# CentaureaHO/CTC-VR

Hardware: AMD Instinct MI355X
Metric: audio-frames/sec, streaming RNN-T greedy decode (higher is better)
Workload: dtype bf16x3; 1 GPU; configs[1]: batch=64/GPU synthetic 10 s 80-dim fbank, streaming chunk=16 (online_rnnt_decode.py semantics), greedy decode, whole-utterance call (tokens identical to the per-chunk API); streams_per_gpu=64, chunk_frames=16, chunks=62, weights=seeded synthetic (seed 0, blank_bias 12.0), parallelism=streams sharded x1, no data-path collective

## Files before the change

ctc-vr_amd/csrc/api_lifecycle.hip.inc:

```

int rnnt_abi_version(void) { return 3; }

const char* rnnt_last_error(const rnnt_ctx* ctx) { return ctx ? ctx->err.c_str() : "null context"; }

int rnnt_create(const rnnt_config* cfg, rnnt_ctx** out) {
    if (!cfg || !out) return RNNT_ERR_ARG;
    *out = nullptr;
    rnnt_ctx* ctx = new rnnt_ctx();
    ctx->cfg = *cfg;
    *out = ctx;
    if (cfg->max_streams < 1 || cfg->max_chunk_frames < 7 || cfg->max_cache_frames < 1 || cfg->max_cache_frames > RNNT_PE_LEN ||
        cfg->max_enc_frames < 1 || cfg->max_tokens < 1 || cfg->vocab_size < 2 || cfg->blank_id < 0 || cfg->blank_id >= cfg->vocab_size ||
        cfg->n_steps < 1 || cfg->max_beam < 0 || cfg->max_beam > 64)
        return fail(ctx, RNNT_ERR_ARG, "rnnt_create: bad config");
    HIPCHK(hipSetDevice(cfg->device));
    if (const char* ng = getenv("RNNT_NO_GRAPH")) ctx->use_graphs = (ng[0] == '1') ? 0 : 1;
    if (const char* pe = getenv("RNNT_PERSISTENT")) ctx->use_persistent = (pe[0] == '0') ? 0 : 1;
    if (const char* me = getenv("RNNT_DEC_MULTI")) ctx->use_multi = (me[0] == '0') ? 0 : 1;
    HIPCHK(hipDeviceGetAttribute(&ctx->n_cus, hipDeviceAttributeMultiprocessorCount, cfg->device));
    if (const char* ae = getenv("RNNT_ATTN_STREAM")) ctx->attn_stream = (ae[0] == '0') ? 0 : 1;
    if (const char* be = getenv("RNNT_BEAM_CHAIN")) ctx->use_beam_chain = (be[0] == '0') ? 0 : 1;
    if (const char* pg = getenv("RNNT_PREFIX_GROUP")) ctx->prefix_group = pg[0] == '1' ? 1 : (pg[0] == '4' ? 4 : 0);
    if (const char* fu = getenv("RNNT_FUSED")) ctx->use_fused = atoi(fu);
    if (const char* fe = getenv("RNNT_FUSE_AFTER_NORM")) ctx->fuse_after_norm = (fe[0] == '0') ? 0 : 1;
    if (const char* me = getenv("RNNT_WF_MERGE")) { const int m = atoi(me); ctx->wf_merge = m < 1 ? 1 : (m > WF_MERGE_MAX ? WF_MERGE_MAX : m); }
    if (const char* le = getenv("RNNT_LM")) ctx->use_lm = (le[0] == '0') ? 0 : 1;
    if (const char* ae2 = getenv("RNNT_AS")) ctx->use_as = (ae2[0] == '0') ? 0 : 1;
    if (const char* e_ = getenv("RNNT_LM_PW2_HEAD")) ctx->lm_pw2_head = atoi(e_);
    if (const char* e_ = getenv("RNNT_LM_FFN_MERGE")) ctx->lm_ffn_merge = atoi(e_);
    if (const char* e_ = getenv("RNNT_LM_SIDE")) ctx->lm_side = atoi(e_);
    if (const char* e_ = getenv("RNNT_LM_QKV_TAIL")) ctx->lm_qkv_tail = atoi(e_);
    if (const char* e_ = getenv("RNNT_LM_OUT_CHAIN")) ctx->lm_out_chain = atoi(e_);
    if (const char* e_ = getenv("RNNT_ATTN_BF")) ctx->attn_bf = atoi(e_);
    if (const char* e_ = getenv("RNNT_ATTN_RESIDENT")) ctx->attn_resident = atoi(e_);
    if (const char* e_ = getenv("RNNT_CONV1_FUSE")) ctx->conv1_fuse = atoi(e_);
    if (const char* se = getenv("RNNT_WF_SUB_ASYNC")) ctx->wf_sub_async = (se[0] == '0') ? 0 : 1;
    const int B = cfg->max_streams;
    ctx->slot = std::vector<PoolSlot>((size_t)B);
    ctx->hs_buf = std::vector<DevBuf<float>>((size_t)B);
    ctx->tmax = sub_len(cfg->max_chunk_frames);
    ctx->t1max = sub1_len(cfg->max_chunk_frames);
    ctx->cap = RNNT_LORDER + WF_MERGE_MAX * ctx->tmax;
    ctx->tcap = cfg->max_cache_frames;
    ctx->fcap = cfg->max_enc_frames;
    ctx->fstride = ctx->fcap + 1;
    ctx->vpad = (cfg->vocab_size + 31) / 32 * 32;
    const size_t M = (size_t)B * ctx->tmax;
    int rc;
#define ALLOC(p, n) if ((rc = reserve(ctx, ctx->p, (size_t)(n)))) return rc
    ALLOC(y1, (size_t)B * ctx->t1max * RNNT_F1 * D);
    ALLOC(y2, M * RNNT_FSUB * D);
    ALLOC(x, M * D);
    ALLOC(hbuf, M * FF);
    ALLOC(qbuf, M * D);
    ALLOC(abuf, M * D);
    ALLOC(dbuf, M * D);
    ALLOC(kcache, (size_t)L * B * ctx->tcap * D);
    ALLOC(vcache, (size_t)L * B * ctx->tcap * D);
    ALLOC(gring, (size_t)L * B * ctx->cap * D);
    ALLOC(xring, (size_t)L * B * ctx->cap * D);
    ALLOC(encbuf, (size_t)B * ctx->fstride * D);
    ALLOC(encp, (size_t)B * ctx->fstride * D);
    ALLOC(h, (size_t)2 * B * D); ALLOC(c, (size_t)2 * B * D); ALLOC(sel, B); ALLOC(key, B);
    ALLOC(pred, (size_t)B * D); ALLOC(z, (size_t)B * D); ALLOC(logits, (size_t)B * ctx->vpad);
    ALLOC(tok, B); ALLOC(fidx, B); ALLOC(nsym, B); ALLOC(count, B); ALLOC(tokens, (size_t)B * cfg->max_tokens);
    ALLOC(n_active, 4); ALLOC(klen, B); ALLOC(dec_ctrl, 32);
    ALLOC(gm_dbg, 16);
    ALLOC(gm_x1, (size_t)2 * B * GM_PARTS * GM_X1);
    ALLOC(gm_xa, (size_t)2 * B * GM_PARTS * 2 * GREEDY_KF);
    if (cfg->max_beam > 0) {
        ctx->max_rows = B * cfg->max_beam;
        const size_t R = ctx->max_rows, NS = cfg->n_steps, KB = cfg->max_beam;
        ALLOC(pool[0], R * (NS + 1) * 512); ALLOC(pool[1], R * (NS + 1) * 512);
        ALLOC(bpred, R * D); ALLOC(bz, R * D); ALLOC(blogits, R * ctx->vpad);
        ALLOC(b_blank, R * NS); ALLOC(b_toplp, R * NS * KB); ALLOC(b_toptok, R * NS * KB);
        ALLOC(b_tok, R); ALLOC(b_frame, R); ALLOC(b_active, R); ALLOC(b_steps, R); ALLOC(b_srcrow, R); ALLOC(b_srcstep, R);
    }
    ALLOC(scratch, std::max((size_t)L * RNNT_H * ctx->tcap * 128, (size_t)B * ctx->fstride * D));
    ALLOC(pinned, 16);
#undef ALLOC
    HIPCHK(hipMemset(ctx->encbuf, 0, (size_t)B * ctx->fstride * D * sizeof(float)));
    HIPCHK(hipMemset(ctx->encp, 0, (size_t)B * ctx->fstride * D * sizeof(float)));
    return RNNT_OK;
}

void rnnt_destroy(rnnt_ctx* ctx) {
    if (ctx) delete ctx;
}

int64_t rnnt_live_device_bytes(void) { return live_device_bytes.load(); }

int rnnt_load_tensor(rnnt_ctx* ctx, const char* name, const float* host_data, int32_t ndim, const int64_t* dims) {
    if (!ctx || !name || ndim < 0 || ndim > 8) return fail(ctx, RNNT_ERR_ARG, "rnnt_load_tensor: bad argument");
    std::string n(name);
    if (n.find("num_batches_tracked") != std::string::npos) return RNNT_OK;
    if (!host_data) return fail(ctx, RNNT_ERR_ARG, "rnnt_load_tensor(%s): null data", name);
    HostTensor t;
    size_t cnt = 1;
    for (int i = 0; i < ndim; ++i) {
        if (dims[i] < 0) return fail(ctx, RNNT_ERR_SHAPE, "rnnt_load_tensor(%s): negative dim", name);
        t.dims.push_back(dims[i]);
        cnt *= (size_t)dims[i];
    }
    t.data.assign(host_data, host_data + cnt);
    ctx->host[n] = std::move(t);
    ctx->finalized = false;
    return RNNT_OK;
}

int rnnt_load_packed(rnnt_ctx* ctx, const float* blob, int64_t n_floats, int32_t on_device, int32_t n_tensors, const char* const* names,
                     const int32_t* ndims, const int64_t* dims_flat) {
    if (!ctx || !blob || !names || !ndims || !dims_flat || n_floats < 0 || n_tensors < 1) return fail(ctx, RNNT_ERR_ARG, "rnnt_load_packed: bad argument");
    std::vector<float> host;
    const float* src = blob;
    if (on_device) {
        HIPCHK(hipSetDevice(ctx->cfg.device));
        host.resize((size_t)n_floats);
        HIPCHK(hipMemcpy(host.data(), blob, (size_t)n_floats * sizeof(float), hipMemcpyDeviceToHost));
        src = host.data();
    }
// ... 365 lines not shown
```

ctc-vr_amd/csrc/host_decode.hip.inc:

```

namespace {

GreedyState greedy_state(rnnt_ctx* ctx) {
    return GreedyState{ctx->tok, ctx->fidx, ctx->nsym, ctx->count, ctx->tokens, ctx->sel, ctx->key, ctx->n_active, ctx->pinned + 8};
}

int greedy_steps_raw(rnnt_ctx* ctx, hipStream_t s, int n) {
    const int B = ctx->n_streams, V = ctx->cfg.vocab_size;
    const long long bs = (long long)ctx->cfg.max_streams * D;
    GreedyState st = greedy_state(ctx);
    int rc;
    for (int it = 0; it < n; ++it) {
        hipLaunchKernelGGL(greedy_decide, dim3(1), dim3(64), 0, s, B, ctx->cfg.blank_id, ctx->cfg.n_steps, ctx->cfg.max_tokens, 0, st);
        LAUNCHCHK("greedy_decide");
        GemmP g1 = plain_gemm(ctx->h, D, ctx->whh_il, D, nullptr, ctx->h, D, B, 4 * D, D, EPI_LSTM);
        g1.X = ctx->egate; g1.I = ctx->tok; g1.X2 = ctx->c; g1.Y2 = ctx->c;
        g1.Asel = ctx->sel; g1.asel_stride = bs; g1.asel_invert = 0;
        g1.act_idx = ctx->fidx; g1.act_lim = ctx->n_active + 2;
        if ((rc = launch_gemm(ctx, s, &g1, 1, TAG_LSTM))) return rc;
        GemmP g3 = plain_gemm(ctx->h, D, ctx->wjc, D, ctx->bjc, ctx->z, D, B, D, D, EPI_TANH_ADD);
        g3.Asel = ctx->sel; g3.asel_stride = bs; g3.asel_invert = 1;
        g3.X = ctx->encp; g3.I = ctx->fidx; g3.x_n = 1; g3.x_s0 = (long long)ctx->fstride * D; g3.x_s1 = D;
        g3.act_idx = ctx->fidx; g3.act_lim = ctx->n_active + 2;
        if ((rc = launch_gemm(ctx, s, &g3, 1, TAG_JOINT_TANH))) return rc;
// ... 32 lines not shown
    e = hipGraphInstantiate(&exec, graph, nullptr, nullptr, 0);
    (void)hipGraphDestroy(graph);
    if (e != hipSuccess) return fail(ctx, RNNT_ERR_HIP, "hipGraphInstantiate failed: %s", hipGetErrorString(e));
    ctx->dec_graphs.push_back({ctx->n_streams, n, exec});
    HIPCHK(hipGraphLaunch(exec, s));
    ctx->launches += 4 * n;
    return RNNT_OK;
}

int greedy_drain(rnnt_ctx* ctx, hipStream_t s, int n_frames, int done_steps) {
    hipLaunchKernelGGL(fill_i32, dim3(1), dim3(64), 0, s, ctx->n_active + 2, n_frames, 1LL);
    LAUNCHCHK("fill_i32");
    const int max_steps = (n_frames - ctx->frames_decoded) * (ctx->cfg.n_steps + 1) + 8;
    int rc;
    while (true) {
        hipLaunchKernelGGL(greedy_decide, dim3(1), dim3(64), 0, s, ctx->n_streams, ctx->cfg.blank_id, ctx->cfg.n_steps, ctx->cfg.max_tokens, 1,
                           greedy_state(ctx));
        LAUNCHCHK("greedy_decide");
        HIPCHK(hipMemcpyAsync(ctx->pinned, ctx->n_active, sizeof(int), hipMemcpyDeviceToHost, s));
        HIPCHK(hipStreamSynchronize(s));
        if (ctx->pinned[0] <= 0) break;
        if (done_steps > max_steps) return fail(ctx, RNNT_ERR_STATE, "greedy decode did not terminate");
        static const int dstep = getenv("RNNT_DRAIN_STEPS") ? atoi(getenv("RNNT_DRAIN_STEPS")) : 4;
        if ((rc = greedy_steps(ctx, s, dstep, n_frames))) return rc;
        done_steps += dstep;
    }
    return RNNT_OK;
}


DecP dec_params(const rnnt_ctx* ctx, int n_total, int n_steps_override, const int* nlim, const int* slots, int n_rows) {
    DecP d{};
    d.whh = ctx->whh_il; d.egate = ctx->egate; d.wjc = ctx->wjc; d.bjc = ctx->bjc; d.wout = ctx->wout; d.bout = ctx->bout;
    d.encp = ctx->encp; d.h = ctx->h; d.c = ctx->c; d.sel = ctx->sel; d.tok = ctx->tok; d.fidx = ctx->fidx; d.nsym = ctx->nsym;
    d.count = ctx->count; d.tokens = ctx->tokens; d.ctrl = ctx->dec_ctrl;
    d.fstride_f = (long long)ctx->fstride * D; d.bstride = (long long)ctx->cfg.max_streams * D;
    d.B = slots ? n_rows : ctx->n_streams; d.vocab = ctx->cfg.vocab_size; d.blank = ctx->cfg.blank_id;
    d.n_steps = n_steps_override > 0 ? n_steps_override : ctx->cfg.n_steps;
    d.max_tokens = ctx->cfg.max_tokens; d.n_total = n_total; d.nlim = nlim; d.slots = slots;
    d.timeout_ticks = 500000000ll;
    return d;
}

bool multi_decoder_ok(const rnnt_ctx* ctx, int rows) {
    return ctx->use_multi && GM_PARTS * rows <= ctx->n_cus && (ctx->cfg.vocab_size + GM_PARTS - 1) / GM_PARTS <= 128;
}

int launch_multi_decoder(rnnt_ctx* ctx, hipStream_t s, const DecP& common) {
    static const bool gdbg = getenv("RNNT_GM_DBG") != nullptr;
    const int B = common.B, rows_per = (common.vocab + GM_PARTS - 1) / GM_PARTS;
    const DecMP d{common, ctx->gm_x1, ctx->gm_xa, rows_per, gdbg ? ctx->gm_dbg : nullptr};
    HIPCHK(hipMemsetAsync(ctx->gm_x1, 0, (size_t)2 * B * GM_PARTS * GM_X1 * sizeof(unsigned long long), s));
    HIPCHK(hipMemsetAsync(ctx->gm_xa, 0, (size_t)2 * B * GM_PARTS * 2 * GREEDY_KF * sizeof(unsigned long long), s));
    const size_t lds = ((size_t)rows_per * GM_WLD + 4 * D + GREEDY_KF * D + 16 * GREEDY_KF + GM_PARTS * 2 * GREEDY_KF + 8 + GREEDY_KF * 4 * 128) * sizeof(float);
    { const int rc_attr = ensure_dyn_lds(ctx, reinterpret_cast<const void*>(&greedy_multi<GREEDY_KF>), 160 * 1024); if (rc_attr) return rc_attr; }
    hipLaunchKernelGGL(greedy_multi<GREEDY_KF>, dim3((unsigned)((B + 7) / 8 * 8 * GM_PARTS)), dim3(512), lds, s, d);
    LAUNCHCHK("greedy_multi");
    return RNNT_OK;
}

int launch_persistent_decoder(rnnt_ctx* ctx, hipStream_t s, int n_total, int n_steps_override = 0, const int* nlim = nullptr,
                              const int* slots = nullptr, int n_rows = 0) {
    const DecP d = dec_params(ctx, n_total, n_steps_override, nlim, slots, n_rows);
    if (multi_decoder_ok(ctx, d.B)) return launch_multi_decoder(ctx, s, d);
    hipLaunchKernelGGL(greedy_stream<GREEDY_KF>, dim3(d.B), dim3(512), 0, s, d);
    LAUNCHCHK("greedy_stream");
    return RNNT_OK;
}

int init_decoder_ctrl(rnnt_ctx* ctx, hipStream_t s, int frames_ready) {
    hipLaunchKernelGGL(fill_i32, dim3(1), dim3(64), 0, s, ctx->dec_ctrl, 0, 32LL);
    LAUNCHCHK("fill_i32");
    hipLaunchKernelGGL(publish_frames, dim3(1), dim3(1), 0, s, ctx->dec_ctrl, frames_ready);
    LAUNCHCHK("publish_frames");
    return RNNT_OK;
}

int probe_overlap(rnnt_ctx* ctx, hipStream_t s, hipStream_t s2) {
    hipLaunchKernelGGL(fill_i32, dim3(1), dim3(64), 0, s, ctx->dec_ctrl, 0, 32LL);
    LAUNCHCHK("fill_i32");
    HIPCHK(hipStreamSynchronize(s));
    hipLaunchKernelGGL(probe_overlap_wait, dim3(1), dim3(1), 0, s2, ctx->dec_ctrl, 2000000LL);
    LAUNCHCHK("probe_overlap_wait");
    hipLaunchKernelGGL(publish_frames, dim3(1), dim3(1), 0, s, ctx->dec_ctrl, 1);
    LAUNCHCHK("publish_frames");
    HIPCHK(hipStreamSynchronize(s2));
    HIPCHK(hipStreamSynchronize(s));
    int r[2] = {0, 0};
    HIPCHK(hipMemcpy(r, ctx->dec_ctrl, sizeof(r), hipMemcpyDeviceToHost));
    ctx->overlap_ok = r[1] ? 1 : 0;
    if (!ctx->overlap_ok)
        fprintf(stderr, "[rnnt] kernels of two HIP streams do not overlap here (serialising profiler or shared hardware queue): "
                        "the resident decoder is replaced by launched evaluation batches\n");
    return RNNT_OK;
}

int finish_persistent_decoder(rnnt_ctx* ctx, hipStream_t s) {
    HIPCHK(hipMemcpyAsync(ctx->pinned + 12, ctx->dec_ctrl, 4 * sizeof(int), hipMemcpyDeviceToHost, s));
    HIPCHK(hipStreamSynchronize(s));
    ctx->greedy_steps += ctx->pinned[14];
    if (getenv("RNNT_GM_DBG") && multi_decoder_ok(ctx, ctx->n_streams)) {
        long long t[16];
        (void)hipMemcpy(t, ctx->gm_dbg, sizeof(t), hipMemcpyDeviceToHost);
        const double ev = t[8] > 0 ? (double)t[8] : 1.0, sy = t[9] > 0 ? (double)t[9] : 1.0;
        fprintf(stderr, "[greedy_multi] stream 0: %lld passes, %lld symbols; us per pass: frames %.2f, decide-tail %.2f, z+logits %.2f, wait XA %.2f; "
                        "us per symbol: W_hh %.2f, cell+W_c %.2f, wait X1 %.2f\n",
                t[8], t[9], t[0] / ev / 100.0, t[6] / ev / 100.0, t[4] / ev / 100.0, t[5] / ev / 100.0, t[1] / sy / 100.0, t[2] / sy / 100.0, t[3] / sy / 100.0);
    }
    if (ctx->pinned[13] != 0) return fail(ctx, RNNT_ERR_STATE, "persistent decoder gave up (code %d: 1 = frame wait, 2 = greedy_multi exchange wait)", ctx->pinned[13]);
    return RNNT_OK;
}

int decode_resident(rnnt_ctx* ctx, hipStream_t s, int n_total, const int* nlim = nullptr, const int* slots = nullptr, int n_rows = 0, int n_steps = 0) {
    int rc;
    if ((rc = init_decoder_ctrl(ctx, s, n_total))) return rc;
    if ((rc = launch_persistent_decoder(ctx, s, n_total, n_steps, nlim, slots, n_rows))) return rc;
    return finish_persistent_decoder(ctx, s);
}

}
```

ctc-vr_amd/csrc/rnnt_api.hip:

```cpp
#include "rnnt_kernels.hip.h"
#include "../../include/rnnt_hip.h"

#include <climits>
#include <cmath>
#include <cstdarg>
#include <cstdio>
#include <chrono>
#include <cstdlib>
#include <cstring>
#include <functional>
#include <map>
#include <string>
#include <unordered_map>
#include <algorithm>
#include <array>
#include <atomic>
#include <vector>

namespace {

constexpr int D = RNNT_D, FF = RNNT_FF, L = RNNT_L, DK = RNNT_DK;
constexpr int BIG = INT_MAX;

struct LayerW {
// ... 94 lines not shown
    PinnedBuf<int> host;
    hipEvent_t ev = nullptr;
    ~CallTab() { if (ev) (void)hipEventDestroy(ev); }
    operator int*() const { return dev.p; }
};

enum WfType { WF_FFN1M, WF_FFN2M, WF_QKV, WF_OUT, WF_PW1, WF_PW2, WF_FFN1, WF_FFN2, WF_ATTN, WF_DW, WF_LN, WF_BLOCK_FRONT, WF_BLOCK_BACK };

}

struct rnnt_ctx {
    rnnt_config cfg;
    std::string err;
    std::map<std::string, HostTensor> host;
    bool finalized = false;
    int numerics = 0;

    DevBuf<float> blob;
    DevBuf<unsigned short> blob_hi, blob_lo;
    DevBuf<uint4> fuse_w;
    DevBuf<LayerDev> layers_dev;
    const uint4* conv2_wp = nullptr;
    DevBuf<unsigned char> joint_wfrag;
    DevBuf<int> joint_counter;
    std::map<const void*, int> dyn_lds;
    std::vector<LayerDev> layers_host;
    int use_as = 1;
    int use_fused = 1;
    DevBuf<FuseItem> wf_ftab;
    int wf_fused_plan = 0;
    LayerW lw[L];
    DevBuf<float> ptab[L];
    const float *conv1_wt, *conv1_b, *conv2_w, *conv2_b, *emb_w, *emb_b, *pe, *after_g, *after_b;
    const float *ln_conv_g_all, *ln_conv_b_all, *glu0;
    const float *whh_il, *wih_il, *b_lstm_il, *pred_embed, *wpr, *bpr, *wenc, *benc, *wpf, *bpf, *wout, *bout;
    DevBuf<float> egate;

    int tmax = 0, t1max = 0, cap = 0, tcap = 0, fcap = 0, fstride = 0, vpad = 0;
    DevBuf<float> y1, y2, x, hbuf, qbuf, abuf, dbuf;
    DevBuf<float> kcache, vcache, gring, xring;
    DevBuf<float> encbuf, encp;
    DevBuf<float> h, c, pred, z, logits;
    DevBuf<int> tok, fidx, nsym, count, tokens, n_active, klen, sel;
    DevBuf<unsigned long long> key;
    DevBuf<int> dec_ctrl;
    int use_persistent = 1;
    int attn_stream = 1;
    int fuse_after_norm = 1;
    int overlap_ok = -1;
    int use_multi = 1;
    int n_cus = 0;
    DevBuf<unsigned long long> gm_x1, gm_xa;
    DevBuf<long long> gm_dbg;
    const float *wjc = nullptr, *bjc = nullptr;
    const float *wctc = nullptr, *bctc = nullptr;
    int max_rows = 0;
    DevBuf<float> pool[2], bpred, bz, blogits, b_blank, b_toplp;
    DevBuf<int> b_tok, b_frame, b_active, b_steps, b_toptok, b_srcrow, b_srcstep;
    int pool_cur = 0;
    PinnedBuf<int> pinned;
    DevBuf<float> scratch;

    int n_streams = 0;
    SlotPos pos{0, 0, 0};
    int frames_buffered = 0, frames_decoded = 0;
    int64_t launches = 0, greedy_steps = 0;
    std::vector<PoolSlot> slot;
    bool pool_mode = false;
    CallTab pool_tab;
    int gemm_m_cap = 0;
    DevBuf<float> wf_x, wf_h, wf_q, wf_a, wf_d, wf_y1, wf_y2;
    int wf_slab = 0;
    DevBuf<int> wf_starts;
    DevBuf<GemmP> wf_gtab; DevBuf<AttnP> wf_atab; DevBuf<DwP> wf_dtab; DevBuf<LnP> wf_ltab;
    hipStream_t dec_stream = nullptr;
    hipStream_t sub_stream = nullptr;
    int wf_sub_async = 1;
    int wf_merge = 2;
    struct WfLaunch { WfType type; int off, n, maxM, maxT2; };
    std::vector<WfLaunch> wf_seq;
    std::vector<std::array<int, 13>> wf_lstart;
    std::vector<int> wf_sc_first, wf_key;
    std::vector<hipEvent_t> ev_pool;
    int use_lm = 1;
    int lm_pw2_head = 2;
    int lm_ffn_merge = 0;
    int lm_qkv_tail = 1, lm_out_chain = 1;
    int lm_side = 1;
    int attn_bf = 1;
    int attn_resident = 1;
    int conv1_fuse = 1;
    DevBuf<float> lm_x, lm_h, lm_q, lm_a, lm_d, lm_g, lm_y1, lm_y2;
    DevBuf<float> lm_y1b, lm_y2b;
    hipEvent_t sub_ev[2] = {nullptr, nullptr};
    DevBuf<float> rg_fb, rg_xt;
    DevBuf<int2> rg_ent;
    DevBuf<LmBlock> lm_blocks;
    std::vector<LmBlock> lm_blocks_host;
    std::vector<int> lm_key;
    DevBuf<LmResHdr> lm_rhdr;
    DevBuf<LmRow> lm_rrows;
    std::vector<LmResHdr> lm_rhdr_host;
    std::vector<LmRow> lm_rrows_host;
    int lm_res_ok = 0, lm_res_stride = 0;
    struct Hyp { std::vector<int> tokens; double log_prob; };
    std::vector<std::vector<Hyp>> beams;
// ... 93 lines not shown
```

ctc-vr_amd/csrc/rnnt_decode.hip.h:

```cpp
#pragma once

struct GreedyState {
    int* tok;
    int* fidx;
    int* nsym;
    int* count;
    int* tokens;
    int* sel;
    unsigned long long* key;
    int* misc;
    int* host_backlog;
};

__global__ __launch_bounds__(64) void greedy_decide(int B, int blank, int n_steps, int max_tokens, int do_count, GreedyState st) {
    const int n_frames = st.misc[2];
    int act = 0, behind = 0;
    for (int b = threadIdx.x; b < B; b += 64) {
        const unsigned long long k64 = st.key[b];
        int f = st.fidx[b];
        if (k64 != 0ull) {
            st.key[b] = 0ull;
            const int k = (int)(0xFFFFFFFFu - (unsigned)(k64 & 0xFFFFFFFFull));
            if (k == blank) {
                f += 1;
// ... 212 lines not shown
            if (nsym >= p.n_steps) { nsym = 0; fidx += 1; }
            commit = true;
            break;
        }
        if (commit) {
            if (tid < RNNT_D) { hs[0][tid] = h2[0][tid]; cs[tid] = c2[tid]; }
            dirty = true;
        }
        ++evals;
        __syncthreads();
    }
    if (tid < RNNT_D) {
        stg1(p.h + (long long)b * RNNT_D + tid, hs[0][tid]);
        stg1(p.c + (long long)b * RNNT_D + tid, cs[tid]);
    }
    if (tid == 0) {
        p.sel[b] = 0; p.tok[b] = tok; p.fidx[b] = p.slots ? 0 : fidx; p.nsym[b] = nsym; p.count[b] = count;
        atomicAdd(p.ctrl + 2, evals);
    }
}

__global__ void unpack_keys(const unsigned long long* __restrict__ key, int* __restrict__ out, long long n) {
    for (long long i = (long long)blockIdx.x * blockDim.x + threadIdx.x; i < n; i += (long long)gridDim.x * blockDim.x)
        out[i] = (int)(0xFFFFFFFFu - (unsigned)(key[i] & 0xFFFFFFFFull));
}

__global__ void publish_frames(int* ctrl, int n) {
    __hip_atomic_store(ctrl, n, __ATOMIC_RELAXED, __HIP_MEMORY_SCOPE_AGENT);
}

__global__ void probe_overlap_wait(int* ctrl, long long ticks) {
    const long long t0 = (long long)__builtin_amdgcn_s_memrealtime();
    int seen = 0;
    while ((long long)__builtin_amdgcn_s_memrealtime() - t0 < ticks) {
        if (__hip_atomic_load(ctrl, __ATOMIC_RELAXED, __HIP_MEMORY_SCOPE_AGENT) != 0) { seen = 1; break; }
        __builtin_amdgcn_s_sleep(32);
    }
    ctrl[1] = seen;
}


__device__ __forceinline__ int ld_sc1i(const int* p) { return __hip_atomic_load(p, __ATOMIC_RELAXED, __HIP_MEMORY_SCOPE_AGENT); }
__device__ __forceinline__ void st_sc1i(int* p, int v) { __hip_atomic_store(p, v, __ATOMIC_RELAXED, __HIP_MEMORY_SCOPE_AGENT); }
__device__ __forceinline__ unsigned long long ld_tag(const unsigned long long* p) {
    return __hip_atomic_load(p, __ATOMIC_RELAXED, __HIP_MEMORY_SCOPE_AGENT);
}
__device__ __forceinline__ void st_tag(unsigned long long* p, unsigned payload, unsigned tag) {
    __hip_atomic_store(p, ((unsigned long long)tag << 32) | payload, __ATOMIC_RELAXED, __HIP_MEMORY_SCOPE_AGENT);
}

#define GM_PARTS 4
#define GM_X1 320
#define GM_WLD 260
struct DecMP : DecP {
    unsigned long long* x1;
    unsigned long long* xa;
    int rows_per;
    long long* dbg;
};

__device__ __forceinline__ bool gm_poll(const DecMP& p, const unsigned long long* src, unsigned tag, unsigned& out) {
    unsigned long long v = ld_tag(src);
    if ((unsigned)(v >> 32) == tag) { out = (unsigned)v; return true; }
    const long long t0 = (long long)__builtin_amdgcn_s_memrealtime();
    int it = 0;
    while (true) {
        v = ld_tag(src);
        if ((unsigned)(v >> 32) == tag) { out = (unsigned)v; return true; }
        if ((++it & 63) == 0) {
            if (ld_sc1i(p.ctrl + 4) != 0) return false;
            if ((long long)__builtin_amdgcn_s_memrealtime() - t0 > p.timeout_ticks) {
                st_sc1i(p.ctrl + 1, 2);
                st_sc1i(p.ctrl + 4, 1);
                return false;
            }
        }
    }
}

#ifndef GM_WHH_REGS
#define GM_WHH_REGS 1
#endif
template <int KF>
__global__ __launch_bounds__(512) void greedy_multi(DecMP p) {
    extern __shared__ __attribute__((aligned(16))) float gm_smem[];
    float* Wo = gm_smem;
    float* hs = Wo + p.rows_per * GM_WLD;
    float* h2 = hs + RNNT_D;
    float* pp = h2 + RNNT_D;
    float* mypp = pp + RNNT_D;
    float* zs = mypp + RNNT_D;
    float* redv = zs + KF * RNNT_D;
    int* redi = reinterpret_cast<int*>(redv + 8 * KF);
    unsigned* xav = reinterpret_cast<unsigned*>(redi + 8 * KF);
    int* s_bad = reinterpret_cast<int*>(xav + GM_PARTS * 2 * KF);
    float* lpart = reinterpret_cast<float*>(s_bad + 4);
    static_assert(KF == 4, "thread (frame, row) mapping of the logit finish assumes KF * 128 == 512");
    const int tid0 = threadIdx.x;
    const int xcd = blockIdx.x & 7, slot = blockIdx.x >> 3;
    const int bi = (slot >> 2) * 8 + xcd, pw = slot & 3;
    if (bi >= p.B) return;
    const int b = p.slots ? ldgi(p.slots + bi) : bi;
    const int cell_unit = 64 * pw + (tid0 >> 3);
    const bool cell = (tid0 & 7) == 0;
    const int v0 = p.rows_per * pw;
    float cc = 0.f, cc2 = 0.f;
    float* gates = zs;
#if GM_WHH_REGS
    float whh_r[128];
    {
        const float* src = p.whh + (long long)(256 * pw + (tid0 >> 1)) * RNNT_D + 128 * (tid0 & 1);
#pragma unroll
        for (int j = 0; j < 32; ++j) {
            const float4 v = ldg4(src + 4 * j);
            whh_r[4 * j] = v.x; whh_r[4 * j + 1] = v.y; whh_r[4 * j + 2] = v.z; whh_r[4 * j + 3] = v.w;
        }
    }
#endif
    float4 wcv[8];
    {
        const float* wc = p.wjc + (long long)(tid0 >> 1) * RNNT_D + 64 * pw + 32 * (tid0 & 1);
#pragma unroll
        for (int u = 0; u < 8; ++u) wcv[u] = ldg4(wc + 4 * u);
    }
    {
    const int tid = tid0;
    for (int e = tid; e < p.rows_per * 64; e += 512) {
        const int r = e >> 6, c4 = (e & 63) * 4;
        const int vr = v0 + r;
        *reinterpret_cast<float4*>(&Wo[r * GM_WLD + c4]) = vr < p.vocab ? ldg4(p.wout + (long long)vr * RNNT_D + c4) : make_float4(0.f, 0.f, 0.f, 0.f);
    }
    const long long soff = (long long)(ldgi(p.sel + b) & 1) * p.bstride + (long long)b * RNNT_D;
    if (tid < RNNT_D) hs[tid] = ldg1(p.h + soff + tid);
    cc = cell ? ldg1(p.c + soff + cell_unit) : 0.f;
    cc2 = cc;
    if (tid == 0) *s_bad = 0;
    }
    int tok = ldgi(p.tok + b), fidx = p.slots ? 0 : ldgi(p.fidx + b), nsym = ldgi(p.nsym + b), count = ldgi(p.count + b);
    const int n_total = p.nlim ? min(p.n_total, ldgi(p.nlim + b)) : p.n_total;
    const float* encp = p.encp + (long long)b * p.fstride_f;
    unsigned long long* x1b = p.x1 + (long long)bi * GM_PARTS * GM_X1;
    unsigned long long* xab = p.xa + (long long)bi * GM_PARTS * 2 * KF;
    const long long x1par = (long long)p.B * GM_PARTS * GM_X1, xapar = (long long)p.B * GM_PARTS * 2 * KF;
    unsigned ev1 = 0, ev3 = 0;
    int evals = 0, seen_ready = 0;
    bool dirty = true, bad = false;
    long long tacc[8] = {0, 0, 0, 0, 0, 0, 0, 0}, tl = (long long)__builtin_amdgcn_s_memrealtime();
    const bool tdbg = p.dbg != nullptr && b == 0 && pw == 0 && tid0 == 0;
#define GM_T(k) { if (tdbg) { const long long t_ = (long long)__builtin_amdgcn_s_memrealtime(); tacc[k] += t_ - tl; tl = t_; } }
    int nsymev = 0;
    __syncthreads();
    while (fidx < n_total) {
        int tid = tid0;
        asm volatile("" : "+v"(tid));
        const int lane = tid & 63, wave = tid >> 6, row2 = tid >> 1, kh = tid & 1;
        (void)lane;
        int avail = seen_ready;
        if (avail <= fidx) {
            if (tid == 0) {
                int nf = ld_sc1i(p.ctrl);
                const long long t0 = (long long)__builtin_amdgcn_s_memrealtime();
                int err = 0;
                while (nf <= fidx) {
                    if (ld_sc1i(p.ctrl + 4) != 0 || (long long)__builtin_amdgcn_s_memrealtime() - t0 > p.timeout_ticks) {
                        st_sc1i(p.ctrl + 1, 1);
                        st_sc1i(p.ctrl + 4, 1);
                        err = 1;
                        break;
                    }
                    __builtin_amdgcn_s_sleep(16);
                    nf = ld_sc1i(p.ctrl);
                }
                __builtin_amdgcn_fence(__ATOMIC_ACQUIRE, "agent");
                redi[0] = err ? -1 : nf;
            }
            __syncthreads();
            avail = redi[0];
            __syncthreads();
            if (avail < 0) { bad = true; break; }
            seen_ready = avail;
        }
        const int kf = dirty ? 1 : min(KF, min(avail, n_total) - fidx);
        float er[KF * RNNT_D / 512];
#pragma unroll
        for (int i2 = 0; i2 < KF * RNNT_D / 512; ++i2) {
            const int e = tid + 512 * i2, k = e >> 8;
            er[i2] = k < kf ? ldg1(encp + (long long)(fidx + k) * RNNT_D + (e & 255)) : 0.f;
        }
        GM_T(0)
        if (dirty) {
            ++nsymev;
            ++ev1;
            unsigned long long* xw = x1b + (ev1 & 1) * x1par;
#if GM_WHH_REGS
            {
                const float eg = ldg1(p.egate + (long long)tok * (4 * RNNT_D) + 256 * pw + row2);
                float a0 = 0.f, a1 = 0.f, a2 = 0.f, a3 = 0.f;
#pragma unroll
                for (int j = 0; j < 32; ++j) {
                    const float4 hv = *reinterpret_cast<const float4*>(&hs[128 * kh + 4 * j]);
                    a0 = fmaf(whh_r[4 * j], hv.x, a0);
                    a1 = fmaf(whh_r[4 * j + 1], hv.y, a1);
                    a2 = fmaf(whh_r[4 * j + 2], hv.z, a2);
                    a3 = fmaf(whh_r[4 * j + 3], hv.w, a3);
                    if ((j & 3) == 3) __builtin_amdgcn_sched_barrier(0);
                }
                float g = (a0 + a1) + (a2 + a3);
                g += __shfl_xor(g, 1, 64);
                if (!kh) gates[row2] = g + eg;
            }
#else
            {
                const float* eg = p.egate + (long long)tok * (4 * RNNT_D) + 256 * pw;
                dec_matvec<1, 512, 4>(p.whh + (long long)(256 * pw) * RNNT_D, RNNT_D, reinterpret_cast<const float (*)[RNNT_D]>(hs),
                                      [&](int n, const float* acc) { gates[n] = acc[0] + ldg1(eg + n); });
            }
#endif
            __syncthreads();
            GM_T(1)
            if (cell) {
                const int unit = 64 * pw + (tid >> 3);
                const float4 gt = *reinterpret_cast<const float4*>(&gates[4 * (tid >> 3)]);
                cc2 = sigmoidf_(gt.y) * cc + sigmoidf_(gt.x) * tanhf(gt.z);
                const float hn = sigmoidf_(gt.w) * tanhf(cc2);
                h2[unit] = hn;
                st_tag(xw + pw * GM_X1 + (unit - 64 * pw), __float_as_uint(hn), ev1);
            }
            __syncthreads();
            {
                float q0 = 0.f, q1 = 0.f;
#pragma unroll
                for (int u = 0; u < 8; ++u) {
                    const float4 hv = *reinterpret_cast<const float4*>(&h2[64 * pw + 32 * kh + 4 * u]);
                    q0 = fmaf(wcv[u].x, hv.x, q0);
                    q1 = fmaf(wcv[u].y, hv.y, q1);
                    q0 = fmaf(wcv[u].z, hv.z, q0);
                    q1 = fmaf(wcv[u].w, hv.w, q1);
                }
                float part = q0 + q1;
                part += __shfl_xor(part, 1, 64);
                if (!kh) {
                    mypp[row2] = part;
                    st_tag(xw + pw * GM_X1 + 64 + row2, __float_as_uint(part), ev1);
                }
            }
            __syncthreads();
            GM_T(2)
            if (tid < RNNT_D) {
                float sum = 0.f;
#pragma unroll
                for (int q = 0; q < GM_PARTS; ++q) {
                    float v = mypp[tid];
                    if (q != pw) {
                        unsigned w = 0;
                        if (!gm_poll(p, xw + q * GM_X1 + 64 + tid, ev1, w)) bad = true;
                        v = __uint_as_float(w);
                    }
                    sum = q == 0 ? v : sum + v;
                }
                pp[tid] = sum + ldg1(p.bjc + tid);
            } else if (tid < RNNT_D + 192) {
                const int idx = tid - RNNT_D;
                int q = idx >> 6;
                if (q >= pw) ++q;
                unsigned w = 0;
                if (!gm_poll(p, xw + q * GM_X1 + (idx & 63), ev1, w)) bad = true;
                h2[64 * q + (idx & 63)] = __uint_as_float(w);
            }
            if (bad) *s_bad = 1;
            __syncthreads();
            if (*s_bad) { bad = true; break; }
            dirty = false;
            GM_T(3)
        }
#pragma unroll
        for (int i2 = 0; i2 < KF * RNNT_D / 512; ++i2) {
            const int e = tid + 512 * i2, k = e >> 8;
            zs[e] = k < kf ? tanhf(pp[e & 255] + er[i2]) : 0.f;
        }
        __syncthreads();
        {
            const int r = tid & 127, qk = tid >> 7;
            if (r < p.rows_per) {
                const float* wl = &Wo[r * GM_WLD + 64 * qk];
#pragma unroll
                for (int k = 0; k < KF; ++k) {
                    if (k < kf) {
                        const float* zk = &zs[k * RNNT_D + 64 * qk];
                        float a0 = 0.f, a1 = 0.f;
#pragma unroll
                        for (int j = 0; j < 16; ++j) {
                            const float4 w = *reinterpret_cast<const float4*>(wl + 4 * j);
                            const float4 z = *reinterpret_cast<const float4*>(zk + 4 * j);
                            a0 = fmaf(w.x, z.x, a0);
                            a1 = fmaf(w.y, z.y, a1);
                            a0 = fmaf(w.z, z.z, a0);
                            a1 = fmaf(w.w, z.w, a1);
                            if ((j & 3) == 3) __builtin_amdgcn_sched_barrier(0);
                        }
                        lpart[(k * 4 + qk) * 128 + r] = a0 + a1;
                    }
                }
            }
        }
        __syncthreads();
        {
            const int k = tid >> 7, r = tid & 127;
            const int vr = v0 + r;
            const bool vin = k < kf && r < p.rows_per && vr < p.vocab;
            float v = -INFINITY;
            int ix = 0x7fffffff;
            if (vin) {
                v = ((lpart[(k * 4) * 128 + r] + lpart[(k * 4 + 1) * 128 + r]) + (lpart[(k * 4 + 2) * 128 + r] + lpart[(k * 4 + 3) * 128 + r])) + ldg1(p.bout + vr);
                ix = vr;
            }
#define GM_STEP(O_) { const float ov = xor_partner<O_>(v); const int oi = __builtin_bit_cast(int, xor_partner<O_>(__builtin_bit_cast(float, ix))); \
                      if (ov > v || (ov == v && oi < ix)) { v = ov; ix = oi; } }
            GM_STEP(1) GM_STEP(2) GM_STEP(4) GM_STEP(8) GM_STEP(16) GM_STEP(32)
#undef GM_STEP
            if (lane == 0) { redv[wave] = v; redi[wave] = ix; }
        }
        __syncthreads();
        GM_T(4)
        ++ev3;
        unsigned long long* xq = xab + (ev3 & 1) * xapar;
        if (tid < KF) {
            float v = redv[2 * tid];
            int ix = redi[2 * tid];
            {
                const float ov = redv[2 * tid + 1];
                const int oi = redi[2 * tid + 1];
                if (ov > v || (ov == v && oi < ix)) { v = ov; ix = oi; }
            }
            unsigned u = 0u;
            if (ix != 0x7fffffff) {
                u = __float_as_uint(v);
                u = (u & 0x80000000u) ? ~u : (u | 0x80000000u);
            }
            st_tag(xq + pw * 2 * KF + 2 * tid, u, ev3);
            st_tag(xq + pw * 2 * KF + 2 * tid + 1, (unsigned)ix, ev3);
            xav[pw * 2 * KF + 2 * tid] = u;
            xav[pw * 2 * KF + 2 * tid + 1] = (unsigned)ix;
        } else if (tid >= 64 && tid < 64 + (GM_PARTS - 1) * 2 * KF) {
            const int idx = tid - 64;
            int q = idx / (2 * KF);
            const int w = idx - q * 2 * KF;
            if (q >= pw) ++q;
            unsigned val = 0;
            if (!gm_poll(p, xq + q * 2 * KF + w, ev3, val)) *s_bad = 1;
            xav[q * 2 * KF + w] = val;
        }
        __syncthreads();
        GM_T(5)
        if (*s_bad) { bad = true; break; }
        bool commit = false;
        for (int k = 0; k < kf; ++k) {
            unsigned bv = 0u;
            int w = 0x7fffffff;
#pragma unroll
            for (int q = 0; q < GM_PARTS; ++q) {
                const unsigned v = xav[q * 2 * KF + 2 * k];
                const int ix = (int)xav[q * 2 * KF + 2 * k + 1];
                if (v > bv || (v == bv && ix < w)) { bv = v; w = ix; }
            }
            if (w == p.blank) { fidx += 1; nsym = 0; continue; }
            if (pw == 0 && tid == 0 && count < p.max_tokens) p.tokens[(long long)b * p.max_tokens + count] = w;
            count += 1;
            tok = w;
            nsym += 1;
            if (nsym >= p.n_steps) { nsym = 0; fidx += 1; }
            commit = true;
            break;
        }
        __syncthreads();
        if (commit) {
            if (tid < RNNT_D) hs[tid] = h2[tid];
            cc = cc2;
            dirty = true;
            __syncthreads();
        }
        ++evals;
        GM_T(6)
    }
    if (tdbg) {
        for (int k = 0; k < 8; ++k) p.dbg[k] = tacc[k];
        p.dbg[8] = evals; p.dbg[9] = nsymev;
    }
#undef GM_T
    if (pw == 0 && tid0 < RNNT_D) stg1(p.h + (long long)b * RNNT_D + tid0, hs[tid0]);
    if (cell) stg1(p.c + (long long)b * RNNT_D + cell_unit, cc);
    if (pw == 0 && tid0 == 0) {
        p.sel[b] = 0; p.tok[b] = tok; p.fidx[b] = p.slots ? 0 : fidx; p.nsym[b] = nsym; p.count[b] = count;
        atomicAdd(p.ctrl + 2, evals);
    }
    (void)bad;
}
```

Measured before the change: 12.84 million audio-frames/s.

## Trim barriers and hoist loads in greedy_multi decode loop, expand per-stream debug timing

Reworks the per-pass loop of the multi-block greedy decoder. The h state now ping-pongs between two LDS buffers chosen by the event parity, which removes the copy and barrier on commit. LSTM gates stay in registers and are swapped between lanes by shuffle, so the shared gates array and its barrier go away. The joint tanh for the first frame is fused into the dirty path, and bias values are hoisted out of the loop. When kf==1 the argmax runs in a single wave with DPP broadcasts, skipping the cross-wave reduction barrier. The debug timing is widened to per-stream rows with dirty/non-dirty splits, at the cost of a small extra LDS region and more complex parity bookkeeping.

```diff
diff --git a/ctc-vr_amd/csrc/api_lifecycle.hip.inc b/ctc-vr_amd/csrc/api_lifecycle.hip.inc
--- a/ctc-vr_amd/csrc/api_lifecycle.hip.inc
+++ b/ctc-vr_amd/csrc/api_lifecycle.hip.inc
@@ -65,7 +65,7 @@
     ALLOC(pred, (size_t)B * D); ALLOC(z, (size_t)B * D); ALLOC(logits, (size_t)B * ctx->vpad);
     ALLOC(tok, B); ALLOC(fidx, B); ALLOC(nsym, B); ALLOC(count, B); ALLOC(tokens, (size_t)B * cfg->max_tokens);
     ALLOC(n_active, 4); ALLOC(klen, B); ALLOC(dec_ctrl, 32);
-    ALLOC(gm_dbg, 16);
+    ALLOC(gm_dbg, (size_t)B * GM_DBG_W);
     ALLOC(gm_x1, (size_t)2 * B * GM_PARTS * GM_X1);
     ALLOC(gm_xa, (size_t)2 * B * GM_PARTS * 2 * GREEDY_KF);
     if (cfg->max_beam > 0) {
diff --git a/ctc-vr_amd/csrc/host_decode.hip.inc b/ctc-vr_amd/csrc/host_decode.hip.inc
--- a/ctc-vr_amd/csrc/host_decode.hip.inc
+++ b/ctc-vr_amd/csrc/host_decode.hip.inc
@@ -108,7 +108,9 @@
     const DecMP d{common, ctx->gm_x1, ctx->gm_xa, rows_per, gdbg ? ctx->gm_dbg : nullptr};
     HIPCHK(hipMemsetAsync(ctx->gm_x1, 0, (size_t)2 * B * GM_PARTS * GM_X1 * sizeof(unsigned long long), s));
     HIPCHK(hipMemsetAsync(ctx->gm_xa, 0, (size_t)2 * B * GM_PARTS * 2 * GREEDY_KF * sizeof(unsigned long long), s));
-    const size_t lds = ((size_t)rows_per * GM_WLD + 4 * D + GREEDY_KF * D + 16 * GREEDY_KF + GM_PARTS * 2 * GREEDY_KF + 8 + GREEDY_KF * 4 * 128) * sizeof(float);
+    const size_t lds = ((size_t)rows_per * GM_WLD + 4 * D + GREEDY_KF * D + 16 * GREEDY_KF + GM_PARTS * 2 * GREEDY_KF + 8 + GREEDY_KF * 4 * 128) * sizeof(float)
+                       + GM_DBG_W * sizeof(long long);
+    ctx->gm_dbg_rows = gdbg ? B : 0;
     { const int rc_attr = ensure_dyn_lds(ctx, reinterpret_cast<const void*>(&greedy_multi<GREEDY_KF>), 160 * 1024); if (rc_attr) return rc_attr; }
     hipLaunchKernelGGL(greedy_multi<GREEDY_KF>, dim3((unsigned)((B + 7) / 8 * 8 * GM_PARTS)), dim3(512), lds, s, d);
     LAUNCHCHK("greedy_multi");
@@ -155,13 +157,26 @@
     HIPCHK(hipMemcpyAsync(ctx->pinned + 12, ctx->dec_ctrl, 4 * sizeof(int), hipMemcpyDeviceToHost, s));
     HIPCHK(hipStreamSynchronize(s));
     ctx->greedy_steps += ctx->pinned[14];
-    if (getenv("RNNT_GM_DBG") && multi_decoder_ok(ctx, ctx->n_streams)) {
-        long long t[16];
-        (void)hipMemcpy(t, ctx->gm_dbg, sizeof(t), hipMemcpyDeviceToHost);
-        const double ev = t[8] > 0 ? (double)t[8] : 1.0, sy = t[9] > 0 ? (double)t[9] : 1.0;
-        fprintf(stderr, "[greedy_multi] stream 0: %lld passes, %lld symbols; us per pass: frames %.2f, decide-tail %.2f, z+logits %.2f, wait XA %.2f; "
-                        "us per symbol: W_hh %.2f, cell+W_c %.2f, wait X1 %.2f\n",
-                t[8], t[9], t[0] / ev / 100.0, t[6] / ev / 100.0, t[4] / ev / 100.0, t[5] / ev / 100.0, t[1] / sy / 100.0, t[2] / sy / 100.0, t[3] / sy / 100.0);
+    if (ctx->gm_dbg_rows > 0) {
+        const int rows = ctx->gm_dbg_rows;
+        ctx->gm_dbg_rows = 0;
+        std::vector<long long> t((size_t)rows * GM_DBG_W);
+        (void)hipMemcpy(t.data(), ctx->gm_dbg, t.size() * sizeof(long long), hipMemcpyDeviceToHost);
+        int row = 0;
+        const char* want = getenv("RNNT_GM_DBG_STREAM");
+        if (want && atoi(want) >= 0 && atoi(want) < rows) row = atoi(want);
+        else for (int i = 1; i < rows; ++i) if (t[(size_t)i * GM_DBG_W + 24] > t[(size_t)row * GM_DBG_W + 24]) row = i;
+        const long long* r = t.data() + (size_t)row * GM_DBG_W;
+        static const char* const name[10] = {"frames", "W_hh", "cell+W_c", "wait X1", "tanh", "quarter sums", "finish+argmax", "XA store", "wait XA", "tail"};
+        fprintf(stderr, "[greedy_multi] row %d (stream %lld, %lld tokens): %lld dirty + %lld non-dirty passes; us per pass, dirty / non-dirty:", row, r[25], r[24],
+                r[22], r[10]);
+        double sum[2] = {0.0, 0.0};
+        for (int k = 0; k < 10; ++k) {
+            const double d = r[12 + k] / 100.0 / (double)(r[22] > 0 ? r[22] : 1), n = r[k] / 100.0 / (double)(r[10] > 0 ? r[10] : 1);
+            sum[0] += d; sum[1] += n;
+            fprintf(stderr, " %s %.2f / %.2f,", name[k], d, n);
+        }
+        fprintf(stderr, " total %.2f / %.2f\n", sum[0], sum[1]);
     }
     if (ctx->pinned[13] != 0) return fail(ctx, RNNT_ERR_STATE, "persistent decoder gave up (code %d: 1 = frame wait, 2 = greedy_multi exchange wait)", ctx->pinned[13]);
     return RNNT_OK;
diff --git a/ctc-vr_amd/csrc/rnnt_api.hip b/ctc-vr_amd/csrc/rnnt_api.hip
--- a/ctc-vr_amd/csrc/rnnt_api.hip
+++ b/ctc-vr_amd/csrc/rnnt_api.hip
@@ -170,6 +170,7 @@
     int n_cus = 0;
     DevBuf<unsigned long long> gm_x1, gm_xa;
     DevBuf<long long> gm_dbg;
+    int gm_dbg_rows = 0;
     const float *wjc = nullptr, *bjc = nullptr;
     const float *wctc = nullptr, *bctc = nullptr;
     int max_rows = 0;
diff --git a/ctc-vr_amd/csrc/rnnt_decode.hip.h b/ctc-vr_amd/csrc/rnnt_decode.hip.h
--- a/ctc-vr_amd/csrc/rnnt_decode.hip.h
+++ b/ctc-vr_amd/csrc/rnnt_decode.hip.h
@@ -288,6 +288,7 @@
 #define GM_PARTS 4
 #define GM_X1 320
 #define GM_WLD 260
+#define GM_DBG_W 32
 struct DecMP : DecP {
     unsigned long long* x1;
     unsigned long long* xa;
@@ -320,10 +321,10 @@
 template <int KF>
 __global__ __launch_bounds__(512) void greedy_multi(DecMP p) {
     extern __shared__ __attribute__((aligned(16))) float gm_smem[];
-    float* Wo = gm_smem;
-    float* hs = Wo + p.rows_per * GM_WLD;
-    float* h2 = hs + RNNT_D;
-    float* pp = h2 + RNNT_D;
+    long long* tsh = reinterpret_cast<long long*>(gm_smem);
+    float* Wo = gm_smem + 2 * GM_DBG_W;
+    float* hb = Wo + p.rows_per * GM_WLD;
+    float* pp = hb + 2 * RNNT_D;
     float* mypp = pp + RNNT_D;
     float* zs = mypp + RNNT_D;
     float* redv = zs + KF * RNNT_D;
@@ -341,7 +342,9 @@
     const bool cell = (tid0 & 7) == 0;
     const int v0 = p.rows_per * pw;
     float cc = 0.f, cc2 = 0.f;
+#if !GM_WHH_REGS
     float* gates = zs;
+#endif
 #if GM_WHH_REGS
     float whh_r[128];
     {
@@ -367,30 +370,36 @@
         *reinterpret_cast<float4*>(&Wo[r * GM_WLD + c4]) = vr < p.vocab ? ldg4(p.wout + (long long)vr * RNNT_D + c4) : make_float4(0.f, 0.f, 0.f, 0.f);
     }
     const long long soff = (long long)(ldgi(p.sel + b) & 1) * p.bstride + (long long)b * RNNT_D;
-    if (tid < RNNT_D) hs[tid] = ldg1(p.h + soff + tid);
+    if (tid < RNNT_D) hb[tid] = ldg1(p.h + soff + tid);
     cc = cell ? ldg1(p.c + soff + cell_unit) : 0.f;
     cc2 = cc;
     if (tid == 0) *s_bad = 0;
-    }
+    if (tid < GM_DBG_W) tsh[tid] = 0;
+    }
+    const int rfin = tid0 & 127;
+    const float bout_r = (rfin < p.rows_per && v0 + rfin < p.vocab) ? ldg1(p.bout + v0 + rfin) : 0.f;
+    const float bout_h = (tid0 < 64 && tid0 + 64 < p.rows_per && v0 + tid0 + 64 < p.vocab) ? ldg1(p.bout + v0 + tid0 + 64) : 0.f;
+    const float bjc_r = tid0 < RNNT_D ? ldg1(p.bjc + tid0) : 0.f;
     int tok = ldgi(p.tok + b), fidx = p.slots ? 0 : ldgi(p.fidx + b), nsym = ldgi(p.nsym + b), count = ldgi(p.count + b);
     const int n_total = p.nlim ? min(p.n_total, ldgi(p.nlim + b)) : p.n_total;
     const float* encp = p.encp + (long long)b * p.fstride_f;
     unsigned long long* x1b = p.x1 + (long long)bi * GM_PARTS * GM_X1;
     unsigned long long* xab = p.xa + (long long)bi * GM_PARTS * 2 * KF;
-    const long long x1par = (long long)p.B * GM_PARTS * GM_X1, xapar = (long long)p.B * GM_PARTS * 2 * KF;
-    unsigned ev1 = 0, ev3 = 0;
-    int evals = 0, seen_ready = 0;
+    const unsigned x1par = (unsigned)p.B * GM_PARTS * GM_X1, xapar = (unsigned)p.B * GM_PARTS * 2 * KF;
+    unsigned ev1 = 1, ev3 = 0;
+    int seen_ready = 0;
     bool dirty = true, bad = false;
-    long long tacc[8] = {0, 0, 0, 0, 0, 0, 0, 0}, tl = (long long)__builtin_amdgcn_s_memrealtime();
-    const bool tdbg = p.dbg != nullptr && b == 0 && pw == 0 && tid0 == 0;
-#define GM_T(k) { if (tdbg) { const long long t_ = (long long)__builtin_amdgcn_s_memrealtime(); tacc[k] += t_ - tl; tl = t_; } }
-    int nsymev = 0;
+    long long tl = (long long)__builtin_amdgcn_s_memrealtime();
+    const bool tdbg = p.dbg != nullptr && pw == 0 && tid0 == 0;
+#define GM_T(k) { if (tdbg) { const long long t_ = (long long)__builtin_amdgcn_s_memrealtime(); \
+                              (void)__hip_atomic_fetch_add(tsh + (dirty ? 12 : 0) + (k), t_ - tl, __ATOMIC_RELAXED, __HIP_MEMORY_SCOPE_WORKGROUP); tl = t_; } }
     __syncthreads();
     while (fidx < n_total) {
         int tid = tid0;
         asm volatile("" : "+v"(tid));
         const int lane = tid & 63, wave = tid >> 6, row2 = tid >> 1, kh = tid & 1;
-        (void)lane;
+        float* hs = hb + (ev1 & 1 ? 0 : RNNT_D);
+        float* h2 = hb + (ev1 & 1 ? RNNT_D : 0);
         int avail = seen_ready;
         if (avail <= fidx) {
             if (tid == 0) {
@@ -423,11 +432,11 @@
             const int e = tid + 512 * i2, k = e >> 8;
             er[i2] = k < kf ? ldg1(encp + (long long)(fidx + k) * RNNT_D + (e & 255)) : 0.f;
         }
+        if (tdbg) (void)__hip_atomic_fetch_add(tsh + (dirty ? 12 : 0) + 10, 1ll, __ATOMIC_RELAXED, __HIP_MEMORY_SCOPE_WORKGROUP);
         GM_T(0)
         if (dirty) {
-            ++nsymev;
-            ++ev1;
             unsigned long long* xw = x1b + (ev1 & 1) * x1par;
+            float gi = 0.f, gf = 0.f, gg = 0.f, go = 0.f;
 #if GM_WHH_REGS
             {
                 const float eg = ldg1(p.egate + (long long)tok * (4 * RNNT_D) + 256 * pw + row2);
@@ -443,7 +452,10 @@
                 }
                 float g = (a0 + a1) + (a2 + a3);
                 g += __shfl_xor(g, 1, 64);
-                if (!kh) gates[row2] = g + eg;
+                gi = g + eg;
+                gf = xor_partner<2>(gi);
+                go = xor_partner<4>(gi);
+                gg = xor_partner<4>(gf);
             }
 #else
             {
@@ -451,14 +463,17 @@
                 dec_matvec<1, 512, 4>(p.whh + (long long)(256 * pw) * RNNT_D, RNNT_D, reinterpret_cast<const float (*)[RNNT_D]>(hs),
                                       [&](int n, const float* acc) { gates[n] = acc[0] + ldg1(eg + n); });
             }
+            __syncthreads();
+            if (cell) {
+                const float4 gt = *reinterpret_cast<const float4*>(&gates[4 * (tid >> 3)]);
+                gi = gt.x; gf = gt.y; gg = gt.z; go = gt.w;
+            }
 #endif
-            __syncthreads();
             GM_T(1)
             if (cell) {
                 const int unit = 64 * pw + (tid >> 3);
-                const float4 gt = *reinterpret_cast<const float4*>(&gates[4 * (tid >> 3)]);
-                cc2 = sigmoidf_(gt.y) * cc + sigmoidf_(gt.x) * tanhf(gt.z);
-                const float hn = sigmoidf_(gt.w) * tanhf(cc2);
+                cc2 = sigmoidf_(gf) * cc + sigmoidf_(gi) * tanhf(gg);
+                const float hn = sigmoidf_(go) * tanhf(cc2);
                 h2[unit] = hn;
                 st_tag(xw + pw * GM_X1 + (unit - 64 * pw), __float_as_uint(hn), ev1);
             }
@@ -494,7 +509,9 @@
                     }
                     sum = q == 0 ? v : sum + v;
                 }
-                pp[tid] = sum + ldg1(p.bjc + tid);
+                const float ppv = sum + bjc_r;
+                pp[tid] = ppv;
+                zs[tid] = tanhf(ppv + er[0]);
             } else if (tid < RNNT_D + 192) {
                 const int idx = tid - RNNT_D;
                 int q = idx >> 6;
@@ -506,15 +523,17 @@
             if (bad) *s_bad = 1;
             __syncthreads();
             if (*s_bad) { bad = true; break; }
-            dirty = false;
             GM_T(3)
         }
-#pragma unroll
-        for (int i2 = 0; i2 < KF * RNNT_D / 512; ++i2) {
-            const int e = tid + 512 * i2, k = e >> 8;
-            zs[e] = k < kf ? tanhf(pp[e & 255] + er[i2]) : 0.f;
-        }
-        __syncthreads();
+        if (!dirty) {
+#pragma unroll
+            for (int i2 = 0; i2 < KF * RNNT_D / 512; ++i2) {
+                const int e = tid + 512 * i2, k = e >> 8;
+                zs[e] = k < kf ? tanhf(pp[e & 255] + er[i2]) : 0.f;
+            }
+            __syncthreads();
+        }
+        GM_T(4)
         {
             const int r = tid & 127, qk = tid >> 7;
             if (r < p.rows_per) {
@@ -540,44 +559,82 @@
             }
         }
         __syncthreads();
-        {
-            const int k = tid >> 7, r = tid & 127;
-            const int vr = v0 + r;
-            const bool vin = k < kf && r < p.rows_per && vr < p.vocab;
-            float v = -INFINITY;
-            int ix = 0x7fffffff;
-            if (vin) {
-                v = ((lpart[(k * 4) * 128 + r] + lpart[(k * 4 + 1) * 128 + r]) + (lpart[(k * 4 + 2) * 128 + r] + lpart[(k * 4 + 3) * 128 + r])) + ldg1(p.bout + vr);
-                ix = vr;
-            }
+        GM_T(5)
+        ++ev3;
+        unsigned long long* xq = xab + (ev3 & 1) * xapar;
 #define GM_STEP(O_) { const float ov = xor_partner<O_>(v); const int oi = __builtin_bit_cast(int, xor_partner<O_>(__builtin_bit_cast(float, ix))); \
                       if (ov > v || (ov == v && oi < ix)) { v = ov; ix = oi; } }
-            GM_STEP(1) GM_STEP(2) GM_STEP(4) GM_STEP(8) GM_STEP(16) GM_STEP(32)
+        if (kf == 1) {
+            if (wave == 0) {
+                float v = -INFINITY;
+                int ix = 0x7fffffff;
+                if (lane < p.rows_per && v0 + lane < p.vocab) {
+                    v = ((lpart[lane] + lpart[128 + lane]) + (lpart[2 * 128 + lane] + lpart[3 * 128 + lane])) + bout_r;
+                    ix = v0 + lane;
+                }
+                if (lane + 64 < p.rows_per && v0 + lane + 64 < p.vocab) {
+                    const float ov = ((lpart[64 + lane] + lpart[128 + 64 + lane]) + (lpart[2 * 128 + 64 + lane] + lpart[3 * 128 + 64 + lane])) + bout_h;
+                    const int oi = v0 + lane + 64;
+                    if (ov > v || (ov == v && oi < ix)) { v = ov; ix = oi; }
+                }
+#define GM_BCAST(C_, M_) { const float ov = __builtin_bit_cast(float, __builtin_amdgcn_update_dpp(__builtin_bit_cast(int, v), __builtin_bit_cast(int, v), C_, M_, 0xF, false)); \
+                           const int oi = __builtin_amdgcn_update_dpp(ix, ix, C_, M_, 0xF, false); \
+                           if (ov > v || (ov == v && oi < ix)) { v = ov; ix = oi; } }
+                GM_STEP(1) GM_STEP(2) GM_STEP(4) GM_STEP(8) GM_BCAST(0x142, 0xA) GM_BCAST(0x143, 0xC)
+#undef GM_BCAST
+                v = __builtin_bit_cast(float, __builtin_amdgcn_readlane(__builtin_bit_cast(int, v), 63));
+                ix = __builtin_amdgcn_readlane(ix, 63);
+                GM_T(6)
+                if (lane < KF) {
+                    unsigned u = 0u;
+                    if (lane != 0) ix = 0x7fffffff;
+                    if (ix != 0x7fffffff) {
+                        u = __float_as_uint(v);
+                        u = (u & 0x80000000u) ? ~u : (u | 0x80000000u);
+                    }
+                    st_tag(xq + pw * 2 * KF + 2 * lane, u, ev3);
+                    st_tag(xq + pw * 2 * KF + 2 * lane + 1, (unsigned)ix, ev3);
+                    xav[pw * 2 * KF + 2 * lane] = u;
+                    xav[pw * 2 * KF + 2 * lane + 1] = (unsigned)ix;
+                }
+            }
+        } else {
+            {
+                const int k = tid >> 7, r = tid & 127;
+                const bool vin = k < kf && r < p.rows_per && v0 + r < p.vocab;
+                float v = -INFINITY;
+                int ix = 0x7fffffff;
+                if (vin) {
+                    v = ((lpart[(k * 4) * 128 + r] + lpart[(k * 4 + 1) * 128 + r]) + (lpart[(k * 4 + 2) * 128 + r] + lpart[(k * 4 + 3) * 128 + r])) + bout_r;
+                    ix = v0 + r;
+                }
+                GM_STEP(1) GM_STEP(2) GM_STEP(4) GM_STEP(8) GM_STEP(16) GM_STEP(32)
+                if (lane == 0) { redv[wave] = v; redi[wave] = ix; }
+            }
+            __syncthreads();
+            GM_T(6)
+            if (tid < KF) {
+                float v = redv[2 * tid];
+                int ix = redi[2 * tid];
+                {
+                    const float ov = redv[2 * tid + 1];
+                    const int oi = redi[2 * tid + 1];
+                    if (ov > v || (ov == v && oi < ix)) { v = ov; ix = oi; }
+                }
+                unsigned u = 0u;
+                if (ix != 0x7fffffff) {
+                    u = __float_as_uint(v);
+                    u = (u & 0x80000000u) ? ~u : (u | 0x80000000u);
+                }
+                st_tag(xq + pw * 2 * KF + 2 * tid, u, ev3);
+                st_tag(xq + pw * 2 * KF + 2 * tid + 1, (unsigned)ix, ev3);
+                xav[pw * 2 * KF + 2 * tid] = u;
+                xav[pw * 2 * KF + 2 * tid + 1] = (unsigned)ix;
+            }
+        }
 #undef GM_STEP
-            if (lane == 0) { redv[wave] = v; redi[wave] = ix; }
-        }
-        __syncthreads();
-        GM_T(4)
-        ++ev3;
-        unsigned long long* xq = xab + (ev3 & 1) * xapar;
-        if (tid < KF) {
-            float v = redv[2 * tid];
-            int ix = redi[2 * tid];
-            {
-                const float ov = redv[2 * tid + 1];
-                const int oi = redi[2 * tid + 1];
-                if (ov > v || (ov == v && oi < ix)) { v = ov; ix = oi; }
-            }
-            unsigned u = 0u;
-            if (ix != 0x7fffffff) {
-                u = __float_as_uint(v);
-                u = (u & 0x80000000u) ? ~u : (u | 0x80000000u);
-            }
-            st_tag(xq + pw * 2 * KF + 2 * tid, u, ev3);
-            st_tag(xq + pw * 2 * KF + 2 * tid + 1, (unsigned)ix, ev3);
-            xav[pw * 2 * KF + 2 * tid] = u;
-            xav[pw * 2 * KF + 2 * tid + 1] = (unsigned)ix;
-        } else if (tid >= 64 && tid < 64 + (GM_PARTS - 1) * 2 * KF) {
+        GM_T(7)
+        if (tid >= 64 && tid < 64 + (GM_PARTS - 1) * 2 * KF) {
             const int idx = tid - 64;
             int q = idx / (2 * KF);
             const int w = idx - q * 2 * KF;
@@ -587,7 +644,7 @@
             xav[q * 2 * KF + w] = val;
         }
         __syncthreads();
-        GM_T(5)
+        GM_T(8)
         if (*s_bad) { bad = true; break; }
         bool commit = false;
         for (int k = 0; k < kf; ++k) {
@@ -608,26 +665,24 @@
             commit = true;
             break;
         }
-        __syncthreads();
         if (commit) {
-            if (tid < RNNT_D) hs[tid] = h2[tid];
+            ++ev1;
             cc = cc2;
-            dirty = true;
-            __syncthreads();
-        }
-        ++evals;
-        GM_T(6)
+        }
+        GM_T(9)
+        dirty = commit;
     }
     if (tdbg) {
-        for (int k = 0; k < 8; ++k) p.dbg[k] = tacc[k];
-        p.dbg[8] = evals; p.dbg[9] = nsymev;
+        tsh[24] = count; tsh[25] = b;
+        long long* out = p.dbg + (long long)((blockIdx.x >> 5) * 8 + (blockIdx.x & 7)) * GM_DBG_W;
+        for (int k = 0; k < GM_DBG_W; ++k) out[k] = tsh[k];
     }
 #undef GM_T
-    if (pw == 0 && tid0 < RNNT_D) stg1(p.h + (long long)b * RNNT_D + tid0, hs[tid0]);
+    if (pw == 0 && tid0 < RNNT_D) stg1(p.h + (long long)b * RNNT_D + tid0, hb[(ev1 & 1 ? 0 : RNNT_D) + tid0]);
     if (cell) stg1(p.c + (long long)b * RNNT_D + cell_unit, cc);
     if (pw == 0 && tid0 == 0) {
         p.sel[b] = 0; p.tok[b] = tok; p.fidx[b] = p.slots ? 0 : fidx; p.nsym[b] = nsym; p.count[b] = count;
-        atomicAdd(p.ctrl + 2, evals);
+        atomicAdd(p.ctrl + 2, (int)ev3);
     }
     (void)bad;
 }
```

After: 13.53 million audio-frames/s, median of 6. +5.4%, better.
